# 123-code/Distributed-neural-networks

Hardware: AMD Instinct MI355X
Metric: images/sec CIFAR-10 2-stage (higher is better)
Workload: dtype fp32 (bf16x3 split emulation, ~2^-16 per product); 1 GPU; model=cifar10-convnet (cifar_model_parts.py NeuralNetwork), global_batch=65536, parallelism=pp2-colocated, stages=2, microbatches=1, stage0_spare_cus=0, p2p=none, stage_cut=conv|fc (reference split, 16 KiB/img hop)

## Files before the change

### csrc/bindings.cpp

```cpp
#include <pybind11/pybind11.h>
#include <pybind11/stl.h>
#include <hip/hip_runtime.h>
#include <cstdint>

#include "kernels/api.h"
#include "comm/p2p.h"

#include <string>
#include <vector>

namespace py = pybind11;
#define P(x) reinterpret_cast<void*>(static_cast<uintptr_t>(x))
#define CP(x) reinterpret_cast<const void*>(static_cast<uintptr_t>(x))
#define FP(x) reinterpret_cast<float*>(static_cast<uintptr_t>(x))
#define CFP(x) reinterpret_cast<const float*>(static_cast<uintptr_t>(x))
#define IP(x) reinterpret_cast<int*>(static_cast<uintptr_t>(x))
#define CIP(x) reinterpret_cast<const int*>(static_cast<uintptr_t>(x))
#define ST(x) reinterpret_cast<hipStream_t>(static_cast<uintptr_t>(x))
typedef uint64_t u64;

PYBIND11_MODULE(_dnn_hip, m) {
  m.doc() = "distributed_neural_networks_amd HIP/CDNA4 kernels (gfx950)";
  m.attr("arch") = "gfx950";

// ... 43 lines not shown
                         P(part), part_cap, ST(st));
  });
  m.def("gemm_rowstats", [](u64 out, int out_ld, u64 in, int in_ld) {
    return dnn_gemm_rowstats(reinterpret_cast<void*>(static_cast<uintptr_t>(out)), out_ld, CP(in), in_ld);
  });
  m.def("gemm_rowstats_written", []() { return dnn_gemm_rowstats_written(); });
  m.def("gemm_set_epi_prefetch", [](int on) { return dnn_gemm_set_epi_prefetch(on); });
  m.def("gemm_oneshot_ablate", [](u64 A, int lda, u64 Wsh, u64 sw, u64 C, int ldc, int M, int N, int K, int cfg,
                                  int abl, u64 st) {
    return dnn_gemm_oneshot_ablate(CP(A), lda, CP(Wsh), CFP(sw), P(C), ldc, M, N, K, cfg, abl, ST(st));
  });
  m.def("quant_fp8_mx", [](u64 x, int ldx, u64 q, int ldq, u64 sx, int M, int K, int kpad, u64 st) {
    return dnn_quant_fp8_mx(CP(x), ldx, P(q), ldq, P(sx), M, K, kpad, ST(st));
  });
  m.def("layernorm_q8_mx", [](u64 x, int ldx, u64 w, u64 b, u64 q, int ldq, u64 sx, int M, int N, int kpad, float eps,
                              int rms, u64 st) {
    return dnn_layernorm_q8_mx(CP(x), ldx, CFP(w), CFP(b), P(q), ldq, P(sx), M, N, kpad, eps, rms, ST(st));
  });
  m.def("gemm_fp8_mx", [](u64 a, u64 sx, u64 w, u64 sw, u64 c, int ldc, u64 bias, u64 r, int ldr, int M, int N, int Kb,
                          int act, u64 qo, int ldq, u64 sxo, int kpo, u64 st) {
    return dnn_gemm_fp8_mx(CP(a), CP(sx), CP(w), CFP(sw), P(c), ldc, CFP(bias), CP(r), ldr, M, N, Kb, act, P(qo), ldq,
                           P(sxo), kpo, ST(st));
  });
  m.def("gemm_fp8_qkv_scatter_mx", [](u64 a, u64 sx, u64 w, u64 sw, u64 bias, u64 q, u64 kc, u64 vc, u64 pos, int B,
                                      int T, int H, int Hkv, int hd, int S, int Kb, u64 st) {
    return dnn_gemm_fp8_qkv_scatter_mx(CP(a), CP(sx), CP(w), CFP(sw), CFP(bias), P(q), P(kc), P(vc),
                                       reinterpret_cast<const int*>(static_cast<uintptr_t>(pos)), B, T, H, Hkv, hd, S,
                                       Kb, ST(st));
  });
  m.def("argmax_final", [](u64 part, int S, int M, u64 out, u64 out2, u64 pos_inc, u64 st, u64 hist, int hist_ld) {
    return dnn_argmax_final(CP(part), S, M, IP(out), IP(out2), IP(pos_inc), ST(st), IP(hist), hist_ld);
  });
  m.def("gemm_oneshot_sweep", [](u64 A, int lda, u64 Wsh, u64 sw, u64 C, int ldc, int M, int N, int K, int mt, int ntw,
                                 int steps, int splitk, int w8, u64 ws, long long ws_bytes, u64 st) {
    return dnn_gemm_oneshot_sweep(CP(A), lda, CP(Wsh), CFP(sw), P(C), ldc, M, N, K, mt, ntw, steps, splitk, w8, P(ws),
                                  ws_bytes, ST(st));
  });
  m.def("gemm_skinny_sweep", [](u64 A, int lda, u64 W, int ldw, u64 sw, u64 C, int ldc, int M, int N, int K, int nt,
                                int u, int ks, int pipe, int w8, u64 st) {
    return dnn_gemm_skinny_sweep(CP(A), lda, CP(W), ldw, CFP(sw), P(C), ldc, M, N, K, nt, u, ks, pipe, w8, ST(st));
  });
  m.def("gemm_set_tile", [](int tile) { return dnn_gemm_set_tile(tile); });
  m.def("gemm_set_anatomy", [](int bits) { return dnn_gemm_set_anatomy(bits); });
  m.def("gemm_set_skinny_pin", [](int id, int ks, int n, int k) { return dnn_gemm_set_skinny_pin(id, ks, n, k); });
  m.def("gemm_set_half_cost", [](float c) { return dnn_gemm_set_half_cost(c); });
  m.def("gemm_bf16_qkv_scatter", [](u64 A, int lda, u64 W, int ldw, u64 bias, u64 rowstat, u64 colsum, u64 q, u64 kc,
                                    u64 vc, u64 pos, int B, int T, int H, int Hkv, int hd, int S, int K, u64 st) {
    return dnn_gemm_bf16_qkv_scatter(CP(A), lda, CP(W), ldw, CFP(bias), CFP(rowstat), CFP(colsum), P(q), P(kc), P(vc),
                                     CIP(pos), B, T, H, Hkv, hd, S, K, ST(st));
  });
  m.def("gemm_fp8_qkv_scatter", [](u64 A8, u64 sa, u64 W8, u64 sw, u64 bias, u64 q, u64 kc, u64 vc, u64 pos, int B,
                                   int T, int H, int Hkv, int hd, int S, int Kb, u64 st) {
    return dnn_gemm_fp8_qkv_scatter(CP(A8), CFP(sa), CP(W8), CFP(sw), CFP(bias), P(q), P(kc), P(vc), CIP(pos), B, T, H,
                                    Hkv, hd, S, Kb, ST(st));
  });
  m.def("gemm_set_res_prefetch", [](int on) { return dnn_gemm_set_res_prefetch(on); });
  m.def("gemm_set_skinny_max_m", [](int m) { return dnn_gemm_set_skinny_max_m(m); });
  m.def("gemm_fp8_set_tile", [](int tile) { return dnn_gemm_fp8_set_tile(tile); });
  m.def("silu_mul_packed", [](u64 gu, int ld_in, u64 out, int ld_out, int M, int F, u64 st) {
    return dnn_silu_mul_packed(CP(gu), ld_in, P(out), ld_out, M, F, ST(st));
  });
  m.def("cifar_stage0_v4", [](u64 x, u64 out, u64 w1p, u64 b1, u64 w2p, u64 b2, int B, int grid, u64 st) {
    return dnn_cifar_stage0_v4(CFP(x), P(out), CP(w1p), CFP(b1), CP(w2p), CFP(b2), B, grid, ST(st));
  });
  m.def("cifar_set_v4_pt", [](int pt) { return dnn_cifar_set_v4_pt(pt); });
  m.def("cifar_stage0_x3", [](u64 x, u64 out, u64 w1h, u64 w1l, u64 b1, u64 w2h, u64 w2l, u64 b2, int B, int grid,
                              u64 st, int split_out) {
    return dnn_cifar_stage0_x3(CFP(x), FP(out), CP(w1h), CP(w1l), CFP(b1), CP(w2h), CP(w2l), CFP(b2), B, grid,
                               ST(st), split_out);
  }, py::arg("x"), py::arg("out"), py::arg("w1h"), py::arg("w1l"), py::arg("b1"), py::arg("w2h"), py::arg("w2l"),
        py::arg("b2"), py::arg("B"), py::arg("grid"), py::arg("st"), py::arg("split_out") = 0);
  m.def("cifar_s0_set_wide_store", [](int on) { return dnn_cifar_s0_set_wide_store(on); });
  m.def("cifar_s0_set_mfma", [](int v) { return dnn_cifar_s0_set_mfma(v); });
  m.def("cifar_s0_get_mfma", []() { return dnn_cifar_s0_get_mfma(); });
  m.def("cifar_split3", [](u64 a, int lda, u64 o, int ldo, int M, int K, u64 st, int blocked) {
    return dnn_cifar_split3(CFP(a), lda, P(o), ldo, M, K, ST(st), blocked);
  }, py::arg("a"), py::arg("lda"), py::arg("o"), py::arg("ldo"), py::arg("M"), py::arg("K"), py::arg("st"),
        py::arg("blocked") = 0);
  m.def("cifar_fc1_x3", [](u64 a, int lda, u64 wh, u64 wl, int ldw, u64 bias, u64 c, int ldc, int M, int N, int K,
                           u64 st, int a_split) {
    return dnn_cifar_fc1_x3(CFP(a), lda, CP(wh), CP(wl), ldw, CFP(bias), FP(c), ldc, M, N, K, ST(st), a_split);
  }, py::arg("a"), py::arg("lda"), py::arg("wh"), py::arg("wl"), py::arg("ldw"), py::arg("bias"), py::arg("c"),
        py::arg("ldc"), py::arg("M"), py::arg("N"), py::arg("K"), py::arg("st"), py::arg("a_split") = 0);
  m.def("cifar_split_blocked", [](u64 a, u64 o, int M, int K, int dir, u64 st) {
    return dnn_cifar_split_blocked(CFP(a), FP(o), M, K, dir, ST(st));
  });
  m.def("cifar_head_tail_x3", [](u64 hid, u64 w2h, u64 w2l, u64 b2, u64 probs, u64 pred, int B, u64 st) {
    return dnn_cifar_head_tail_x3(CFP(hid), CP(w2h), CP(w2l), CFP(b2), FP(probs), IP(pred), B, ST(st));
  });
  m.def("cifar_head_tail", [](u64 hid, u64 w2p, u64 b2, u64 probs, u64 pred, int B, u64 st) {
    return dnn_cifar_head_tail(CP(hid), CP(w2p), CFP(b2), FP(probs), IP(pred), B, ST(st));
  });
#ifdef DNN_HAVE_TRANSFORMER
  m.def("row_stats", [](u64 x, int ldx, u64 stats, int M, int N, float eps, int rms, u64 st) {
    return dnn_row_stats(CP(x), ldx, FP(stats), M, N, eps, rms, ST(st));
  });
  m.def("layernorm", [](u64 x, int ldx, u64 w, u64 b, u64 y, int ldy, int M, int N, float eps, int rms, u64 st) {
    return dnn_layernorm(CP(x), ldx, CFP(w), CFP(b), P(y), ldy, M, N, eps, rms, ST(st));
  });
  m.def("layernorm_q8", [](u64 x, int ldx, u64 w, u64 b, u64 q, int ldq, u64 sq, int M, int N, int kpad, float eps,
                           int rms, u64 st, int split) {
    return dnn_layernorm_q8(CP(x), ldx, CFP(w), CFP(b), P(q), ldq, FP(sq), M, N, kpad, eps, rms, ST(st), split);
  }, py::arg("x"), py::arg("ldx"), py::arg("w"), py::arg("b"), py::arg("q"), py::arg("ldq"), py::arg("sq"), py::arg("M"),
     py::arg("N"), py::arg("kpad"), py::arg("eps"), py::arg("rms"), py::arg("st"), py::arg("split") = 0);
  m.def("embed_gpt2", [](u64 idx, u64 wte, u64 wpe, u64 out, int B, int T, int d, u64 pos, int V, int Pn, u64 st) {
    return dnn_embed_gpt2(CIP(idx), CP(wte), CP(wpe), P(out), B, T, d, CIP(pos), V, Pn, ST(st));
  });
  m.def("qkv_split", [](u64 qkv, u64 q, u64 kc, u64 vc, int B, int T, int H, int Hkv, int hd, int S, u64 pos,
                        u64 cos, u64 sin, int rope, u64 st, int kv8) {
    return dnn_qkv_split(CP(qkv), P(q), P(kc), P(vc), B, T, H, Hkv, hd, S, CIP(pos), CFP(cos), CFP(sin), rope,
                         ST(st), kv8);
  }, py::arg("qkv"), py::arg("q"), py::arg("kc"), py::arg("vc"), py::arg("B"), py::arg("T"), py::arg("H"),
     py::arg("Hkv"), py::arg("hd"), py::arg("S"), py::arg("pos"), py::arg("cos"), py::arg("sin"), py::arg("rope"),
     py::arg("st"), py::arg("kv8") = 0);
  m.def("flash_attn_qkv", [](u64 qkv, int ldqkv, u64 kc, u64 vc, u64 o, int B, int T, int H, int Hkv, int hd, int S,
                             u64 pos, float scale, u64 st, int kv8) {
    return dnn_flash_attn_qkv(CP(qkv), ldqkv, P(kc), P(vc), P(o), B, T, H, Hkv, hd, S, CIP(pos), scale, ST(st), kv8);
  }, py::arg("qkv"), py::arg("ldqkv"), py::arg("kc"), py::arg("vc"), py::arg("o"), py::arg("B"), py::arg("T"),
     py::arg("H"), py::arg("Hkv"), py::arg("hd"), py::arg("S"), py::arg("pos"), py::arg("scale"), py::arg("st"),
     py::arg("kv8") = 0);
  m.def("flash_attn", [](u64 q, u64 kc, u64 vc, u64 o, int B, int T, int H, int Hkv, int hd, int S, u64 pos,
                         float scale, u64 st, int kv8) {
    return dnn_flash_attn(CP(q), CP(kc), CP(vc), P(o), B, T, H, Hkv, hd, S, CIP(pos), scale, ST(st), kv8);
  }, py::arg("q"), py::arg("kc"), py::arg("vc"), py::arg("o"), py::arg("B"), py::arg("T"), py::arg("H"),
     py::arg("Hkv"), py::arg("hd"), py::arg("S"), py::arg("pos"), py::arg("scale"), py::arg("st"), py::arg("kv8") = 0);
  m.def("attn_decode", [](u64 q, u64 kc, u64 vc, u64 o, int B, int H, int Hkv, int hd, int S, u64 lens,
                          float scale, int splits, u64 ws, u64 st, int kv8) {
    return dnn_attn_decode(CP(q), CP(kc), CP(vc), P(o), B, H, Hkv, hd, S, CIP(lens), scale, splits, FP(ws), ST(st),
                           kv8);
  }, py::arg("q"), py::arg("kc"), py::arg("vc"), py::arg("o"), py::arg("B"), py::arg("H"), py::arg("Hkv"),
     py::arg("hd"), py::arg("S"), py::arg("lens"), py::arg("scale"), py::arg("splits"), py::arg("ws"), py::arg("st"),
     py::arg("kv8") = 0);
  m.def("attn_decode_qkv", [](u64 qkv, int ldqkv, u64 kc, u64 vc, u64 o, int B, int H, int Hkv, int hd, int S,
                              u64 pos, u64 cos, u64 sin, float scale, int splits, u64 ws, u64 st, int kv8) {
    return dnn_attn_decode_qkv(CP(qkv), ldqkv, P(kc), P(vc), P(o), B, H, Hkv, hd, S, CIP(pos), CFP(cos), CFP(sin),
                               scale, splits, FP(ws), ST(st), kv8);
  }, py::arg("qkv"), py::arg("ldqkv"), py::arg("kc"), py::arg("vc"), py::arg("o"), py::arg("B"), py::arg("H"),
     py::arg("Hkv"), py::arg("hd"), py::arg("S"), py::arg("pos"), py::arg("cos"), py::arg("sin"), py::arg("scale"),
     py::arg("splits"), py::arg("ws"), py::arg("st"), py::arg("kv8") = 0);
  m.def("sample_topk", [](u64 x, int ld, int M, int N, u64 out, float temperature, int topk, unsigned seed, u64 step,
                          u64 st) {
    return dnn_sample_topk(CP(x), ld, M, N, reinterpret_cast<int*>(out), temperature, topk, seed,
                           reinterpret_cast<const int*>(step), ST(st));
  });
  m.def("sample_rows", [](u64 x, int ld, int M, int N, u64 out, float temperature, int topk, float top_p, float min_p,
                          unsigned seed, u64 step, u64 st, u64 out2, u64 pos_inc, u64 hist, int hist_ld, u64 thr_out) {
    return dnn_sample_rows(CP(x), ld, M, N, IP(out), temperature, topk, top_p, min_p, seed,
                           reinterpret_cast<const int*>(step), ST(st), IP(out2), IP(pos_inc), IP(hist), hist_ld,
                           IP(thr_out));
  }, py::arg("x"), py::arg("ld"), py::arg("M"), py::arg("N"), py::arg("out"), py::arg("temperature"), py::arg("topk"),
     py::arg("top_p"), py::arg("min_p"), py::arg("seed"), py::arg("step"), py::arg("st"), py::arg("out2") = 0,
     py::arg("pos_inc") = 0, py::arg("hist") = 0, py::arg("hist_ld") = 0, py::arg("thr_out") = 0);
  m.def("argmax_rows", [](u64 x, int ld, int M, int N, u64 out, int f32in, u64 st, u64 out2, u64 pos_inc, u64 part,
                          u64 hist, int hist_ld) {
    return dnn_argmax_rows(CP(x), ld, M, N, IP(out), f32in, ST(st), IP(out2), IP(pos_inc),
                           reinterpret_cast<void*>(static_cast<uintptr_t>(part)), IP(hist), hist_ld);
  }, py::arg("x"), py::arg("ld"), py::arg("M"), py::arg("N"), py::arg("out"), py::arg("f32in"), py::arg("st"),
     py::arg("out2") = 0, py::arg("pos_inc") = 0, py::arg("part") = 0, py::arg("hist") = 0, py::arg("hist_ld") = 0);
  m.def("quant_fp8_rows", [](u64 x, int ldx, u64 q, u64 scale, int M, int K, int kpad, u64 st, int split) {
    return dnn_quant_fp8_rows(CP(x), ldx, P(q), FP(scale), M, K, kpad, ST(st), split);
  }, py::arg("x"), py::arg("ldx"), py::arg("q"), py::arg("scale"), py::arg("M"), py::arg("K"), py::arg("kpad"),
     py::arg("st"), py::arg("split") = 0);
  m.def("gemm_fp8", [](u64 A, u64 sa, u64 W, u64 sw, u64 C, int ldc, u64 bias, u64 R, int ldr, int M, int N, int K,
                       int act, u64 st) {
    return dnn_gemm_fp8(CP(A), CFP(sa), CP(W), CFP(sw), P(C), ldc, CFP(bias), CP(R), ldr, M, N, K, act, ST(st));
  });
// ... 48 lines not shown
```

### csrc/kernels/api.h

```cpp
#pragma once
#include <hip/hip_runtime.h>

extern "C" {
int dnn_gemm_bf16(const void* A, int lda, const void* W, int ldw, void* C, int ldc, const float* bias, const void* R,
                  int ldr, int M, int N, int K, int act, int out_f32, hipStream_t st, const void* Wsh = nullptr,
                  const float* rowstat = nullptr, const float* colsum = nullptr, void* ws = nullptr,
                  long long ws_bytes = 0);
int dnn_row_stats(const void* x, int ldx, float* stats, int M, int N, float eps, int rms, hipStream_t st);
int dnn_gemm_set_tile(int tile);
int dnn_gemm_set_anatomy(int bits);
int dnn_gemm_set_skinny_pin(int id, int ks, int n, int k);
int dnn_gemm_bf16_qkv_scatter(const void* A, int lda, const void* W, int ldw, const float* bias, const float* rowstat,
                              const float* colsum, void* q, void* kc, void* vc, const int* pos, int B, int T, int H,
                              int Hkv, int hd, int S, int K, hipStream_t st);
int dnn_gemm_fp8_qkv_scatter(const void* A8, const float* sa, const void* W8, const float* sw, const float* bias,
                             void* q, void* kc, void* vc, const int* pos, int B, int T, int H, int Hkv, int hd, int S,
                             int Kb, hipStream_t st);
int dnn_gemm_set_res_prefetch(int on);
int dnn_gemm_set_half_cost(float c);
int dnn_gemm_set_skinny_max_m(int m);
int dnn_gemm_fp8_set_tile(int tile);
int dnn_gemm_fp8_256(const void* A, const float* sa, const void* W, const float* sw, void* C, int ldc, const float* bias,
                     const void* R, int ldr, int M, int N, int Kb, int act, hipStream_t st);
int dnn_gemm_skinny_sweep(const void* A, int lda, const void* W, int ldw, const float* sw, void* C, int ldc, int M,
                          int N, int K, int nt, int u, int ks, int pipe, int w8, hipStream_t st);
int dnn_gemm_skinny_norm(const void* A, int lda, const void* W, int ldw, void* C, int ldc, const float* bias,
                         const void* R, int ldr, int M, int N, int K, int act, int norm, const float* colsum, float eps,
                         hipStream_t st, const void* Wsh = nullptr, void* ws = nullptr, long long ws_bytes = 0);
int dnn_gemm_skinny_w8(const void* A, int lda, const void* W, int ldw, const float* sw, void* C, int ldc,
                       const float* bias, const void* R, int ldr, int M, int N, int K, int act, int norm,
                       const float* colsum, float eps, hipStream_t st, const void* Wsh = nullptr, void* ws = nullptr,
                       long long ws_bytes = 0);
int dnn_gemm_skinny(const void* A, int lda, const float* sa, const void* W, int ldw, const float* sw, void* C, int ldc,
                    const float* bias, const void* R, int ldr, int M, int N, int K, int act, int out_f32, int fp8,
                    hipStream_t st, const void* Wsh = nullptr, void* ws = nullptr, long long ws_bytes = 0);
int dnn_gemm_set_stream(int on, long long min_bytes, int fold = -1);
int dnn_gemm_set_oneshot(int on, int mt, int ntw, int steps, int splitk);
int dnn_gemm_set_oneshot_lds_floor(int bytes);
int dnn_gemm_set_oneshot_probe(void* rec, int abl);
int dnn_gemm_oneshot_sweep(const void* A, int lda, const void* Wsh, const float* sw, void* C, int ldc, int M, int N,
                           int K, int mt, int ntw, int steps, int splitk, int w8, void* ws, long long ws_bytes,
                           hipStream_t st);
int dnn_gemm_set_head(int on);
int dnn_gemm_head(const void* A, int lda, const void* Wsh, const float* sw, const float* colsum, const float* bias,
                  float eps, int norm, void* C, int ldc, int M, int N, int K, int w8, void* part, int part_cap,
                  hipStream_t st);
int dnn_argmax_final(const void* part, int S, int M, int* out, int* out2, int* pos_inc, hipStream_t st,
                     int* hist = nullptr, int hist_ld = 0);
int dnn_gemm_set_split_tail(int on);
int dnn_quant_fp8_mx(const void* x, int ldx, void* q, int ldq, void* sx, int M, int K, int kpad, hipStream_t st);
int dnn_layernorm_q8_mx(const void* x, int ldx, const float* w, const float* b, void* q, int ldq, void* sx, int M,
                        int N, int kpad, float eps, int rms, hipStream_t st);
int dnn_gemm_fp8_mx(const void* A8, const void* sx, const void* W8, const float* sw, void* C, int ldc,
                    const float* bias, const void* R, int ldr, int M, int N, int Kb, int act, void* qo, int ldq,
                    void* sxo, int kpo, hipStream_t st);
int dnn_gemm_fp8_qkv_scatter_mx(const void* A8, const void* sx, const void* W8, const float* sw, const float* bias,
                                void* q, void* kc, void* vc, const int* pos, int B, int T, int H, int Hkv, int hd,
                                int S, int Kb, hipStream_t st);
int dnn_gemm_rowstats(void* out, int out_ld, const void* in, int in_ld);
int dnn_gemm_rowstats_written();
int dnn_gemm_set_epi_prefetch(int on);
int dnn_gemm_oneshot_ablate(const void* A, int lda, const void* Wsh, const float* sw, void* C, int ldc, int M, int N,
                            int K, int cfg, int abl, hipStream_t st);
int dnn_silu_mul_packed(const void* gu, int ld_in, void* out, int ld_out, int M, int F, hipStream_t st);
int dnn_cifar_stage0_v4(const float* x, void* out, const void* w1p, const float* b1, const void* w2p, const float* b2,
                        int B, int grid, hipStream_t st);
int dnn_cifar_set_v4_pt(int pt);
int dnn_cifar_stage0_x3(const float* x, float* out, const void* w1h, const void* w1l, const float* b1, const void* w2h,
                        const void* w2l, const float* b2, int B, int grid, hipStream_t st, int split_out = 0);
int dnn_cifar_s0_set_wide_store(int on);
int dnn_cifar_s0_set_mfma(int v);
int dnn_cifar_s0_get_mfma();
int dnn_cifar_split3(const float* a, int lda, void* o, int ldo, int M, int K, hipStream_t st, int blocked = 0);
int dnn_cifar_fc1_x3(const float* A, int lda, const void* Wh, const void* Wl, int ldw, const float* bias, float* C,
                     int ldc, int M, int N, int K, hipStream_t st, int a_split = 0);
int dnn_cifar_split_blocked(const float* a, float* o, int M, int K, int dir, hipStream_t st);
int dnn_cifar_head_tail_x3(const float* hid, const void* w2h, const void* w2l, const float* b2, float* probs, int* pred,
                           int B, hipStream_t st);
int dnn_cifar_head_tail(const void* hid, const void* w2p, const float* b2, float* probs, int* pred, int B,
                        hipStream_t st);
int dnn_layernorm_q8(const void* x, int ldx, const float* w, const float* b, void* q, int ldq, float* sq, int M, int N,
                     int kpad, float eps, int rms, hipStream_t st, int split = 0);
int dnn_layernorm(const void* x, int ldx, const float* w, const float* b, void* y, int ldy, int M, int N, float eps,
                  int rms, hipStream_t st);
int dnn_embed_gpt2(const int* idx, const void* wte, const void* wpe, void* out, int B, int T, int d, const int* pos,
                   int V, int P, hipStream_t st);
int dnn_qkv_split(const void* qkv, void* q, void* kc, void* vc, int B, int T, int H, int Hkv, int hd, int S,
                  const int* pos, const float* cos, const float* sin, int rope, hipStream_t st, int kv8 = 0);
int dnn_flash_attn_qkv(const void* qkv, int ldqkv, void* kc, void* vc, void* o, int B, int T, int H, int Hkv,
                       int hd, int S, const int* pos, float scale, hipStream_t st, int kv8 = 0);
int dnn_flash_attn(const void* q, const void* kc, const void* vc, void* o, int B, int T, int H, int Hkv, int hd, int S,
                   const int* pos, float scale, hipStream_t st, int kv8 = 0);
int dnn_attn_decode_qkv(const void* qkv, int ldqkv, void* kc, void* vc, void* o, int B, int H, int Hkv, int hd, int S,
                        const int* pos, const float* cosT, const float* sinT, float scale, int splits, float* ws,
                        hipStream_t st, int kv8 = 0);
int dnn_attn_decode(const void* q, const void* kc, const void* vc, void* o, int B, int H, int Hkv, int hd, int S,
                    const int* lens, float scale, int splits, float* ws, hipStream_t st, int kv8 = 0);
int dnn_sample_topk(const void* x, int ld, int M, int N, int* out, float temperature, int topk, unsigned seed,
                    const int* step, hipStream_t st);
int dnn_sample_rows(const void* x, int ld, int M, int N, int* out, float temperature, int topk, float top_p,
                    float min_p, unsigned seed, const int* step, hipStream_t st, int* out2 = nullptr,
                    int* pos_inc = nullptr, int* hist = nullptr, int hist_ld = 0, int* thr_out = nullptr);
int dnn_argmax_rows(const void* x, int ld, int M, int N, int* out, int f32in, hipStream_t st, int* out2 = nullptr,
                    int* pos_inc = nullptr, void* part = nullptr, int* hist = nullptr, int hist_ld = 0);
int dnn_quant_fp8_rows(const void* x, int ldx, void* q, float* scale, int M, int K, int kpad, hipStream_t st,
                       int split = 0);
int dnn_gemm_fp8(const void* A, const float* sa, const void* W, const float* sw, void* C, int ldc, const float* bias,
                 const void* R, int ldr, int M, int N, int K, int act, hipStream_t st);
}
```

### csrc/kernels/cifar_x3.hip

```cpp
#include <type_traits>

#include "gemm_epilogue.h"

namespace dnn {
namespace x3 {

__device__ __forceinline__ void split2(float a, float b, uint32_t& hi, uint32_t& lo) {
  hi = pack2bf(a, b);
  const float ah = __uint_as_float(hi << 16), bh = __uint_as_float(hi & 0xffff0000u);
  lo = pack2bf(a - ah, b - bh);
}

__device__ __forceinline__ int dpp_xor1(int v) { return __builtin_amdgcn_mov_dpp(v, 0xB1, 0xF, 0xF, false); }
__device__ __forceinline__ int dpp_xor2(int v) { return __builtin_amdgcn_mov_dpp(v, 0x4E, 0xF, 0xF, false); }

constexpr int XW = 40;
constexpr int XPL = 34 * XW * 8;
constexpr int A1PL = 18 * 18 * 64;
constexpr int A1_OFF = 4 * XPL;
constexpr int LDS_BYTES = A1_OFF + 4 * A1PL;

__device__ __forceinline__ int xin_off(int k, int lo) { return ((k & 1) * 2 + lo) * XPL; }
__device__ __forceinline__ int a1_off(int k, int lo) { return A1_OFF + ((k & 1) * 2 + lo) * A1PL; }

// ... 324 lines not shown
#pragma unroll
          for (int par = 0; par < 2; ++par) b[ky][par] = rb + lb[ky][par];
        f32x16 acc[2] = {f32x16{}, f32x16{}};
        bf16x8 a0[4], a1[4];
        c2_issue<0>(b, a0);
        c2_step<0>(b, w2hf, w2lf, acc, a0, a1);
        if constexpr (WIDE) {
#pragma unroll
          for (int qy = 0; qy < 2; ++qy) {
            const int g0 = (2 * qy) * 4;
            float v[2][2];
#pragma unroll
            for (int i = 0; i < 2; ++i) {
              v[i][0] = fmaxf(fmax_nan(fmax_nan(acc[i][g0], acc[i][g0 + 1]), fmax_nan(acc[i][g0 + 4], acc[i][g0 + 5])) + bias, 0.f);
              v[i][1] = fmaxf(fmax_nan(fmax_nan(acc[i][g0 + 2], acc[i][g0 + 3]), fmax_nan(acc[i][g0 + 6], acc[i][g0 + 7])) + bias,
                              0.f);
            }
            const auto sx = __builtin_amdgcn_permlane32_swap(__float_as_uint(v[0][0]), __float_as_uint(v[1][0]), false,
                                                             false);
            const auto sy = __builtin_amdgcn_permlane32_swap(__float_as_uint(v[0][1]), __float_as_uint(v[1][1]), false,
                                                             false);
            const int PY = 2 * ty2 + qy;
            if constexpr (SPLIT_OUT) {
              uint2 hi, lo;
              split2(__uint_as_float(sx[0]), __uint_as_float(sy[0]), hi.x, lo.x);
              split2(__uint_as_float(sx[1]), __uint_as_float(sy[1]), hi.y, lo.y);
              char* bp = reinterpret_cast<char*>(ob - oc2 * 64) + (oc2 * 2 + (PY >> 2)) * 128 + ((PY & 3) * 8 + 4 * h) * 2;
              *reinterpret_cast<uint2*>(bp) = hi;
              *reinterpret_cast<uint2*>(bp + 64) = lo;
            } else {
              *reinterpret_cast<uint4*>(ob + PY * 8 + 4 * h) = make_uint4(sx[0], sy[0], sx[1], sy[1]);
            }
          }
        } else {
#pragma unroll
        for (int i = 0; i < 2; ++i) {
#pragma unroll
          for (int qy = 0; qy < 2; ++qy) {
            float2 pv;
            const int g0 = (2 * qy) * 4;
            pv.x = fmaxf(fmax_nan(fmax_nan(acc[i][g0], acc[i][g0 + 1]), fmax_nan(acc[i][g0 + 4], acc[i][g0 + 5])) + bias, 0.f);
            pv.y = fmaxf(fmax_nan(fmax_nan(acc[i][g0 + 2], acc[i][g0 + 3]), fmax_nan(acc[i][g0 + 6], acc[i][g0 + 7])) + bias,
                         0.f);
            const int PY = 2 * ty2 + qy, PX = 4 * i + 2 * h;
            if constexpr (SPLIT_OUT) {
              uint32_t hi, lo;
              split2(pv.x, pv.y, hi, lo);
              char* bp = reinterpret_cast<char*>(ob - oc2 * 64) + (oc2 * 2 + (PY >> 2)) * 128 + ((PY & 3) * 8 + PX) * 2;
              *reinterpret_cast<uint32_t*>(bp) = hi;
              *reinterpret_cast<uint32_t*>(bp + 64) = lo;
            } else {
              *reinterpret_cast<float2*>(ob + PY * 8 + PX) = pv;
            }
          }
        }
        }
      }
    };

    __syncthreads();
    for (int it = 0; it <= n; ++it) {
      if (it >= 1) conv2_img(it - 1);
      __syncthreads();
    }
  }
}

constexpr int F1_T = 256, F1_K = 32, F1_PLANE = 256 * 64;

__device__ __forceinline__ int f1_swz(int r) { return (r >> 2) & 2; }

__device__ __forceinline__ bf16x8 f1_frag(const char* plane, int row, int chunk) {
  return *reinterpret_cast<const bf16x8*>(plane + row * 64 + ((chunk ^ f1_swz(row)) << 4));
}

__device__ __forceinline__ void f1_tile_coords(int logical, int ntm, int ntn, int& tm, int& tn) {
  constexpr int G = 8;
  const int per = G * ntn, grp = logical / per, first = grp * G;
  const int gm = min(ntm - first, G), r = logical - grp * per;
  tm = first + r % gm;
  tn = r / gm;
}

template <bool SPLIT_IN>
__global__ __launch_bounds__(512, 1) void cifar_fc1_x3_kernel(const float* __restrict__ A, int lda,
                                                              const bf16_t* __restrict__ Wh,
                                                              const bf16_t* __restrict__ Wl, int ldw,
                                                              const float* __restrict__ bias, float* __restrict__ C,
                                                              int ldc, int M, int N, int K) {
  __shared__ __attribute__((aligned(1024))) char smem[2 * 4 * F1_PLANE];
  const int tid = threadIdx.x, lane = tid & 63, wave = tid >> 6;
  const int ntn = N / F1_T, ntm = (M + F1_T - 1) / F1_T;
  int tm, tn;
  f1_tile_coords(xcd_remap(blockIdx.x, ntm * ntn), ntm, ntn, tm, tn);
  const int m0 = tm * F1_T, n0 = tn * F1_T;
  const int wr = wave >> 2, wc = wave & 3;
  const int nk = K / F1_K;
  auto plane = [&](int u, int p) { return smem + (u * 4 + p) * F1_PLANE; };

  float4 ar[4];
  auto load_a = [&](int t, auto) {
#pragma unroll
    for (int k = 0; k < 4; ++k) {
      const int row = min(m0 + (tid >> 3) + 64 * k, M - 1);
      ar[k] = *reinterpret_cast<const float4*>(A + (size_t)row * lda + t * F1_K + (tid & 7) * 4);
    }
  };
  auto store_a = [&](int u, auto) {
#pragma unroll
    for (int k = 0; k < 4; ++k) {
      const int r = (tid >> 3) + 64 * k, c = (tid & 7) >> 1, half = tid & 1;
      uint2 hi, lo;
      split2(ar[k].x, ar[k].y, hi.x, lo.x);
      split2(ar[k].z, ar[k].w, hi.y, lo.y);
      const int o = r * 64 + ((c ^ f1_swz(r)) << 4) + half * 8;
      *reinterpret_cast<uint2*>(plane(u, 0) + o) = hi;
      *reinterpret_cast<uint2*>(plane(u, 1) + o) = lo;
    }
  };
  auto stage_a = [&](int u, int t) {
    const char* Ab = reinterpret_cast<const char*>(A);
#pragma unroll
    for (int p = 0; p < 2; ++p) {
#pragma unroll
      for (int j = 0; j < 2; ++j) {
        const int piece = wave * 2 + j, rl = piece * 16 + (lane >> 2);
        const int c = (lane & 3) ^ f1_swz(rl);
        const int row = min(m0 + rl, M - 1);
        glds16(Ab + (size_t)row * lda * 4 + t * 128 + p * 64 + c * 16, plane(u, p) + piece * 1024);
      }
    }
  };
  auto stage_w = [&](int u, int t) {
#pragma unroll
    for (int p = 0; p < 2; ++p) {
      const bf16_t* W = p ? Wl : Wh;
#pragma unroll
      for (int j = 0; j < 2; ++j) {
        const int piece = wave * 2 + j, rl = piece * 16 + (lane >> 2);
        const int c = (lane & 3) ^ f1_swz(rl);
        glds16(W + (size_t)(n0 + rl) * ldw + t * F1_K + c * 8, plane(u, 2 + p) + piece * 1024);
      }
    }
  };

  f32x4 acc[8][4];
#pragma unroll
  for (int i = 0; i < 8; ++i)
#pragma unroll
    for (int j = 0; j < 4; ++j) acc[i][j] = f32x4{0.f, 0.f, 0.f, 0.f};

  using I0 = std::integral_constant<int, 0>;
  if constexpr (SPLIT_IN) {
    stage_a(0, 0);
    stage_w(0, 0);
    asm volatile("s_waitcnt vmcnt(0)" ::: "memory");
  } else {
    load_a(0, I0{});
    stage_w(0, 0);
    asm volatile("s_waitcnt vmcnt(0)" ::: "memory");
    store_a(0, I0{});
  }
  __syncthreads();

  const int fr = lane & 15, fc = lane >> 4;
  auto compute = [&](int u) {
    const char* ah_p = plane(u, 0);
    const char* al_p = plane(u, 1);
    const char* bh_p = plane(u, 2);
    const char* bl_p = plane(u, 3);
    bf16x8 bh[4], bl[4];
#pragma unroll
    for (int j = 0; j < 4; ++j) {
      bh[j] = f1_frag(bh_p, wc * 64 + j * 16 + fr, fc);
      bl[j] = f1_frag(bl_p, wc * 64 + j * 16 + fr, fc);
    }
#pragma unroll
    for (int h = 0; h < 2; ++h) {
      bf16x8 ah[4], al[4];
#pragma unroll
      for (int i = 0; i < 4; ++i) {
        ah[i] = f1_frag(ah_p, wr * 128 + (h * 4 + i) * 16 + fr, fc);
        al[i] = f1_frag(al_p, wr * 128 + (h * 4 + i) * 16 + fr, fc);
      }
#pragma unroll
      for (int i = 0; i < 4; ++i)
#pragma unroll
        for (int j = 0; j < 4; ++j) {
          f32x4& a = acc[h * 4 + i][j];
          a = __builtin_amdgcn_mfma_f32_16x16x32_bf16(bh[j], ah[i], a, 0, 0, 0);
          a = __builtin_amdgcn_mfma_f32_16x16x32_bf16(bl[j], ah[i], a, 0, 0, 0);
          a = __builtin_amdgcn_mfma_f32_16x16x32_bf16(bh[j], al[i], a, 0, 0, 0);
        }
    }
  };
  auto barrier = [&]() {
    asm volatile("s_waitcnt lgkmcnt(0)" ::: "memory");
    __builtin_amdgcn_sched_barrier(0);
    __builtin_amdgcn_s_barrier();
    __builtin_amdgcn_sched_barrier(0);
  };
  for (int t = 0; t < nk; ++t) {
    const int u = t & 1;
    if (t + 1 < nk) {
      if constexpr (SPLIT_IN)
        stage_a(u ^ 1, t + 1);
      else
        load_a(t + 1, I0{});
      stage_w(u ^ 1, t + 1);
    }
    compute(u);
    if (t + 1 < nk) {
      asm volatile("s_waitcnt vmcnt(0)" ::: "memory");
      if constexpr (!SPLIT_IN) store_a(u ^ 1, I0{});
    }
    barrier();
  }

  const bool vec = epi_vec_ok(C, ldc, bias, nullptr, 0);
#pragma unroll
  for (int i = 0; i < 8; ++i) {
    const int m = m0 + wr * 128 + i * 16 + fr;
#pragma unroll
    for (int j = 0; j < 4; ++j)
      epi_t4<ACT_RELU, true>(acc[i][j], m, n0 + wc * 64 + j * 16 + fc * 4, M, N, C, ldc, bias, nullptr, 0, vec);
  }
}

__global__ __launch_bounds__(256) void cifar_split_blocked_kernel(const float* __restrict__ a, float* __restrict__ o,
                                                                  int M, int K, int dir) {
  const int per_row = K / 8;
  const long total = (long)M * per_row;
  for (long e = blockIdx.x * 256L + threadIdx.x; e < total; e += (long)gridDim.x * 256) {
    const int m = (int)(e / per_row), k = (int)(e % per_row) * 8;
    char* rowp = reinterpret_cast<char*>(o + (size_t)m * K);
    const char* rowa = reinterpret_cast<const char*>(a + (size_t)m * K);
    const int hoff = (k >> 5) * 128 + (k & 31) * 2;
    if (dir == 0) {
      const float4 u = *reinterpret_cast<const float4*>(rowa + k * 4);
      const float4 v = *reinterpret_cast<const float4*>(rowa + k * 4 + 16);
      uint4 hi, lo;
      split2(u.x, u.y, hi.x, lo.x);
      split2(u.z, u.w, hi.y, lo.y);
      split2(v.x, v.y, hi.z, lo.z);
      split2(v.z, v.w, hi.w, lo.w);
      *reinterpret_cast<uint4*>(rowp + hoff) = hi;
      *reinterpret_cast<uint4*>(rowp + hoff + 64) = lo;
    } else {
      const uint4 hi = *reinterpret_cast<const uint4*>(rowa + hoff);
      const uint4 lo = *reinterpret_cast<const uint4*>(rowa + hoff + 64);
      const uint32_t h[4] = {hi.x, hi.y, hi.z, hi.w}, l[4] = {lo.x, lo.y, lo.z, lo.w};
      float r[8];
#pragma unroll
      for (int i = 0; i < 4; ++i) {
        r[2 * i] = __uint_as_float(h[i] << 16) + __uint_as_float(l[i] << 16);
        r[2 * i + 1] = __uint_as_float(h[i] & 0xffff0000u) + __uint_as_float(l[i] & 0xffff0000u);
      }
      *reinterpret_cast<float4*>(rowp + k * 4) = float4{r[0], r[1], r[2], r[3]};
      *reinterpret_cast<float4*>(rowp + k * 4 + 16) = float4{r[4], r[5], r[6], r[7]};
    }
  }
}

__global__ __launch_bounds__(256) void cifar_split3_kernel(const float* __restrict__ a, int lda,
                                                           bf16_t* __restrict__ o, int ldo, int M, int K,
                                                           int blocked) {
  const int per_row = K / 8;
  const long total = (long)M * per_row;
  for (long e = blockIdx.x * 256L + threadIdx.x; e < total; e += (long)gridDim.x * 256) {
    const int m = (int)(e / per_row), c = (int)(e % per_row) * 8;
    uint4 hi, lo;
    if (blocked) {
      const char* rowa = reinterpret_cast<const char*>(a + (size_t)m * lda) + (c >> 5) * 128 + (c & 31) * 2;
      hi = *reinterpret_cast<const uint4*>(rowa);
      lo = *reinterpret_cast<const uint4*>(rowa + 64);
    } else {
      const float4 u = *reinterpret_cast<const float4*>(a + (size_t)m * lda + c);
      const float4 v = *reinterpret_cast<const float4*>(a + (size_t)m * lda + c + 4);
      split2(u.x, u.y, hi.x, lo.x);
      split2(u.z, u.w, hi.y, lo.y);
      split2(v.x, v.y, hi.z, lo.z);
      split2(v.z, v.w, hi.w, lo.w);
    }
    bf16_t* r = o + (size_t)m * ldo + c;
    *reinterpret_cast<uint4*>(r) = hi;
    *reinterpret_cast<uint4*>(r + K) = hi;
    *reinterpret_cast<uint4*>(r + 2 * K) = lo;
  }
}

__global__ __launch_bounds__(256) void cifar_head_tail_x3_kernel(const float* __restrict__ hid,
                                                                 const bf16_t* __restrict__ w2h,
                                                                 const bf16_t* __restrict__ w2l,
                                                                 const float* __restrict__ b2,
                                                                 float* __restrict__ probs, int* __restrict__ pred,
                                                                 int B) {
  const int lane = threadIdx.x & 63;
  const int gw = (blockIdx.x * blockDim.x + threadIdx.x) >> 6;
  const int nw = (gridDim.x * blockDim.x) >> 6;
// ... 11 lines not shown
    const float* ap = hid + (size_t)rc * 512 + kq;
    f32x4 acc = {0.f, 0.f, 0.f, 0.f};
#pragma unroll
    for (int s = 0; s < 16; ++s) {
      const float4 u = *reinterpret_cast<const float4*>(ap + s * 32);
      const float4 v = *reinterpret_cast<const float4*>(ap + s * 32 + 4);
      uint4 hi, lo;
      split2(u.x, u.y, hi.x, lo.x);
      split2(u.z, u.w, hi.y, lo.y);
      split2(v.x, v.y, hi.z, lo.z);
      split2(v.z, v.w, hi.w, lo.w);
      const bf16x8 ah = __builtin_bit_cast(bf16x8, hi), al = __builtin_bit_cast(bf16x8, lo);
      acc = __builtin_amdgcn_mfma_f32_16x16x32_bf16(ah, wfh[s], acc, 0, 0, 0);
      acc = __builtin_amdgcn_mfma_f32_16x16x32_bf16(ah, wfl[s], acc, 0, 0, 0);
      acc = __builtin_amdgcn_mfma_f32_16x16x32_bf16(al, wfh[s], acc, 0, 0, 0);
    }
#pragma unroll
    for (int r = 0; r < 4; ++r) {
      const float z = col < 10 ? acc[r] + bias : -INFINITY;
      float mx = z;
#pragma unroll
      for (int o = 1; o < 16; o <<= 1) mx = fmaxf(mx, __shfl_xor(mx, o, 64));
      const float e = col < 10 ? expf(z - mx) : 0.f;
      float sum = e;
#pragma unroll
      for (int o = 1; o < 16; o <<= 1) sum += __shfl_xor(sum, o, 64);
      int cand = (z == mx) ? col : 16;
#pragma unroll
      for (int o = 1; o < 16; o <<= 1) cand = min(cand, __shfl_xor(cand, o, 64));
      const int m = r0 + (lane >> 4) * 4 + r;
      if (m < B) {
        if (col < 10) probs[(size_t)m * 10 + col] = e / sum;
        if (col == 0) pred[m] = cand;
      }
    }
  }
}

}

using namespace dnn;

static int g_s0_wide_store = 1;
static int g_s0_mfma = 1;

extern "C" int dnn_cifar_s0_set_mfma(int v) {
  if (v < 0 || v > 1) return 1;
  g_s0_mfma = v;
  return 0;
}

extern "C" int dnn_cifar_s0_get_mfma() { return g_s0_mfma; }

extern "C" int dnn_cifar_s0_set_wide_store(int on) {
  g_s0_wide_store = on ? 1 : 0;
  return 0;
}

template <bool SPLIT_OUT>
static int launch_stage0_x3(const float* x, float* out, const void* w1h, const void* w1l, const float* b1,
                            const void* w2h, const void* w2l, const float* b2, int B, int grid, hipStream_t st) {
  if (g_s0_mfma == 1)
    hipLaunchKernelGGL((cifar_stage0_x3_kernel<true, SPLIT_OUT, 1>), dim3(grid), dim3(512), 0, st, x, out,
                       (const bf16_t*)w1h, (const bf16_t*)w1l, b1, (const bf16_t*)w2h, (const bf16_t*)w2l, b2, B);
  else if (g_s0_wide_store)
    hipLaunchKernelGGL((cifar_stage0_x3_kernel<true, SPLIT_OUT>), dim3(grid), dim3(512), 0, st, x, out,
                       (const bf16_t*)w1h, (const bf16_t*)w1l, b1, (const bf16_t*)w2h, (const bf16_t*)w2l, b2, B);
  else
    hipLaunchKernelGGL((cifar_stage0_x3_kernel<false, SPLIT_OUT>), dim3(grid), dim3(512), 0, st, x, out,
                       (const bf16_t*)w1h, (const bf16_t*)w1l, b1, (const bf16_t*)w2h, (const bf16_t*)w2l, b2, B);
  return (int)hipGetLastError();
}

extern "C" int dnn_cifar_stage0_x3(const float* x, float* out, const void* w1h, const void* w1l, const float* b1,
                                   const void* w2h, const void* w2l, const float* b2, int B, int grid,
                                   hipStream_t st, int split_out) {
  if (B <= 0) return 0;
  if (grid <= 0) grid = 256;
  if (grid > B) grid = B;
  return split_out ? launch_stage0_x3<true>(x, out, w1h, w1l, b1, w2h, w2l, b2, B, grid, st)
                   : launch_stage0_x3<false>(x, out, w1h, w1l, b1, w2h, w2l, b2, B, grid, st);
}

extern "C" int dnn_cifar_fc1_x3(const float* A, int lda, const void* Wh, const void* Wl, int ldw, const float* bias,
                                float* C, int ldc, int M, int N, int K, hipStream_t st, int a_split) {
  if (M <= 0) return 0;
  if (N % F1_T != 0 || K % F1_K != 0 || lda % 4 != 0 || ldw % 8 != 0 || ldc % 4 != 0) return -1;
  const int blocks = ((M + F1_T - 1) / F1_T) * (N / F1_T);
  if (a_split)
    hipLaunchKernelGGL(cifar_fc1_x3_kernel<true>, dim3(blocks), dim3(512), 0, st, A, lda, (const bf16_t*)Wh,
                       (const bf16_t*)Wl, ldw, bias, C, ldc, M, N, K);
  else
    hipLaunchKernelGGL(cifar_fc1_x3_kernel<false>, dim3(blocks), dim3(512), 0, st, A, lda, (const bf16_t*)Wh,
                       (const bf16_t*)Wl, ldw, bias, C, ldc, M, N, K);
  return (int)hipGetLastError();
}

extern "C" int dnn_cifar_split_blocked(const float* a, float* o, int M, int K, int dir, hipStream_t st) {
  if (M <= 0) return 0;
  if (K % 32 != 0 || a == o) return -1;
  const long total = (long)M * (K / 8);
  long blocks = (total + 255) / 256;
  if (blocks > 8192) blocks = 8192;
  hipLaunchKernelGGL(cifar_split_blocked_kernel, dim3((int)blocks), dim3(256), 0, st, a, o, M, K, dir);
  return (int)hipGetLastError();
}

extern "C" int dnn_cifar_split3(const float* a, int lda, void* o, int ldo, int M, int K, hipStream_t st, int blocked) {
  if (M <= 0) return 0;
  if (K % 8 != 0 || lda % 4 != 0 || ldo % 8 != 0 || ldo < 3 * K || (blocked && K % 32 != 0)) return -1;
  const long total = (long)M * (K / 8);
  long blocks = (total + 255) / 256;
  if (blocks > 8192) blocks = 8192;
  hipLaunchKernelGGL(cifar_split3_kernel, dim3((int)blocks), dim3(256), 0, st, a, lda, (bf16_t*)o, ldo, M, K, blocked);
  return (int)hipGetLastError();
}

extern "C" int dnn_cifar_head_tail_x3(const float* hid, const void* w2h, const void* w2l, const float* b2,
                                      float* probs, int* pred, int B, hipStream_t st) {
  if (B <= 0) return 0;
  int waves = (B + 15) / 16;
  int blocks = (waves + 3) / 4;
  if (blocks > 1024) blocks = 1024;
  hipLaunchKernelGGL(cifar_head_tail_x3_kernel, dim3(blocks), dim3(256), 0, st, hid, (const bf16_t*)w2h,
                     (const bf16_t*)w2l, b2, probs, pred, B);
  return (int)hipGetLastError();
}
```

### distributed_neural_networks_amd/ops/cifar.py

```python
from __future__ import annotations

from dataclasses import dataclass
from typing import Dict, Optional, Tuple

import torch

from ._lib import check, lib, ptr, stream_ptr
from .gemm import ACT_RELU, linear

PRECISIONS = ("fp32", "bf16")


def split_bf16(w: torch.Tensor) -> Tuple[torch.Tensor, torch.Tensor]:
    w = w.float()
    hi = w.to(torch.bfloat16)
    lo = (w - hi.float()).to(torch.bfloat16)
    return hi, lo


def _conv1_k48(sd) -> torch.Tensor:
    w = torch.zeros(32, 3, 4, 4)
    w[:, :, :3, :3] = sd["conv1.weight"].float().permute(0, 2, 3, 1)
    return w.reshape(32, 48)

# ... 21 lines not shown
    w2l: torch.Tensor = None


@dataclass
class CifarHeadWeights:
    precision: str
    w_fc1: torch.Tensor = None
    w_fc1h: torch.Tensor = None
    w_fc1l: torch.Tensor = None
    b_fc1: torch.Tensor = None
    w_fc2: torch.Tensor = None
    w_fc2h: torch.Tensor = None
    w_fc2l: torch.Tensor = None
    b_fc2: torch.Tensor = None


def _check_precision(p: str) -> str:
    if p not in PRECISIONS:
        raise ValueError(f"CIFAR precision must be one of {PRECISIONS}, got {p!r}")
    return p


def pack_stage0(sd: Dict[str, torch.Tensor], device, precision: str = "fp32") -> CifarStage0Weights:
    _check_precision(precision)
    b1 = sd["conv1.bias"].float().to(device).contiguous()
    b2 = sd["conv2.bias"].float().to(device).contiguous()
    w1, w2 = _conv1_k48(sd), _conv2_k288(sd)
    if precision == "bf16":
        return CifarStage0Weights("bf16", b1, b2,
                                  w1=w1.to(device=device, dtype=torch.bfloat16).contiguous(),
                                  w2=w2.to(device=device, dtype=torch.bfloat16).contiguous())
    (w1h, w1l), (w2h, w2l) = split_bf16(w1), split_bf16(w2)
    dv = lambda t: t.to(device).contiguous()
    return CifarStage0Weights("fp32", b1, b2, w1h=dv(w1h), w1l=dv(w1l), w2h=dv(w2h), w2l=dv(w2l))


def pack_head(sd: Dict[str, torch.Tensor], device, fc1: bool = True, fc2: bool = True,
              precision: str = "fp32") -> CifarHeadWeights:
    _check_precision(precision)
    w = CifarHeadWeights(precision)
    if fc1:
        f = sd["fc1.weight"].float()
        if precision == "bf16":
            w.w_fc1 = f.to(device=device, dtype=torch.bfloat16).contiguous()
        else:
            hi, lo = split_bf16(f)
            w.w_fc1 = torch.cat([hi, lo, hi], dim=1).to(device).contiguous()
            w.w_fc1h, w.w_fc1l = hi.to(device).contiguous(), lo.to(device).contiguous()
        w.b_fc1 = sd["fc1.bias"].float().to(device).contiguous()
    if fc2:
        f2 = _fc2_pad(sd)
        if precision == "bf16":
            w.w_fc2 = f2.to(device=device, dtype=torch.bfloat16).contiguous()
        else:
            hi, lo = split_bf16(f2)
            w.w_fc2h, w.w_fc2l = hi.to(device).contiguous(), lo.to(device).contiguous()
        w.b_fc2 = sd["fc2.bias"].float().to(device).contiguous()
    return w


def act_dtype(precision: str) -> torch.dtype:
    return torch.float32 if _check_precision(precision) == "fp32" else torch.bfloat16


STAGE0_GRID = 0
FC1_X3_MIN_ROWS = 16384


def set_stage0_grid(grid: int = 0) -> None:
    global STAGE0_GRID
    STAGE0_GRID = int(grid)


STAGE0_MFMA = {"32x32x16": 0, "16x16x32": 1}


def set_stage0_mfma(shape) -> int:
    v = STAGE0_MFMA[shape] if isinstance(shape, str) else int(shape)
    prev = lib().cifar_s0_get_mfma()
    check(lib().cifar_s0_set_mfma(v), "cifar_s0_set_mfma")
    return prev


def _check_act(t: torch.Tensor, shape, dtype, what: str) -> None:
    if t.dtype != dtype or tuple(t.shape[1:]) != tuple(shape) or not t.is_contiguous():
        raise ValueError(f"{what}: expected contiguous {dtype} (B,{','.join(map(str, shape))}), "
                         f"got {t.dtype} {tuple(t.shape)}")


BOUNDARIES = ("fp32", "split")


def _split_boundary(boundary: str, precision: str) -> int:
    if boundary not in BOUNDARIES:
        raise ValueError(f"boundary must be one of {BOUNDARIES}, got {boundary!r}")
    if boundary == "split" and precision != "fp32":
        raise ValueError("the split boundary encoding exists for the fp32 precision only")
    return int(boundary == "split")


def encode_boundary(h: torch.Tensor, out: Optional[torch.Tensor] = None) -> torch.Tensor:
    out = torch.empty_like(h) if out is None else out
    check(lib().cifar_split_blocked(ptr(h), ptr(out), h.shape[0], h.shape[1], 0, stream_ptr()), "encode_boundary")
    return out


def decode_boundary(h: torch.Tensor, out: Optional[torch.Tensor] = None) -> torch.Tensor:
    out = torch.empty_like(h) if out is None else out
    check(lib().cifar_split_blocked(ptr(h), ptr(out), h.shape[0], h.shape[1], 1, stream_ptr()), "decode_boundary")
    return out


def stage0_forward(x: torch.Tensor, w: CifarStage0Weights, out: Optional[torch.Tensor] = None,
                   grid: int = 0, boundary: str = "fp32") -> torch.Tensor:
    split = _split_boundary(boundary, w.precision)
    grid = grid or STAGE0_GRID
    _check_act(x, (3, 32, 32), torch.float32, "stage0 input")
    B = x.shape[0]
    dt = act_dtype(w.precision)
    if out is None:
        out = torch.empty((B, 4096), dtype=dt, device=x.device)
    if tuple(out.shape) != (B, 4096) or out.dtype != dt or not out.is_contiguous():
        raise ValueError("stage0: bad output buffer")
    if w.precision == "fp32":
        check(lib().cifar_stage0_x3(ptr(x), ptr(out), ptr(w.w1h), ptr(w.w1l), ptr(w.b1), ptr(w.w2h), ptr(w.w2l),
                                    ptr(w.b2), B, grid, stream_ptr(), split), "cifar_stage0_x3")
    else:
        check(lib().cifar_stage0_v4(ptr(x), ptr(out), ptr(w.w1), ptr(w.b1), ptr(w.w2), ptr(w.b2), B, grid,
                                    stream_ptr()), "cifar_stage0_v4")
    return out


def fc1_forward(h: torch.Tensor, w: CifarHeadWeights, out: Optional[torch.Tensor] = None,
                scratch: Optional[torch.Tensor] = None, boundary: str = "fp32") -> torch.Tensor:
    split = _split_boundary(boundary, w.precision)
    dt = act_dtype(w.precision)
    _check_act(h, (4096,), dt, "fc1 input")
    B = h.shape[0]
    if w.precision == "bf16":
        return linear(h, w.w_fc1, w.b_fc1, act=ACT_RELU, out=out)
    if B >= FC1_X3_MIN_ROWS:
        if out is None:
            out = torch.empty((B, 512), dtype=torch.float32, device=h.device)
        check(lib().cifar_fc1_x3(ptr(h), 4096, ptr(w.w_fc1h), ptr(w.w_fc1l), 4096, ptr(w.b_fc1), ptr(out), 512,
                                 B, 512, 4096, stream_ptr(), split), "cifar_fc1_x3")
        return out
    if scratch is None or scratch.shape[0] < B or tuple(scratch.shape[1:]) != (3 * 4096,):
        scratch = torch.empty((B, 3 * 4096), dtype=torch.bfloat16, device=h.device)
    a3 = scratch[:B]
    check(lib().cifar_split3(ptr(h), 4096, ptr(a3), 3 * 4096, B, 4096, stream_ptr(), split), "cifar_split3")
    if out is None:
        out = torch.empty((B, 512), dtype=torch.float32, device=h.device)
    return linear(a3, w.w_fc1, w.b_fc1, act=ACT_RELU, out=out)


def head_tail(hid: torch.Tensor, w: CifarHeadWeights, probs: Optional[torch.Tensor] = None,
              pred: Optional[torch.Tensor] = None) -> Tuple[torch.Tensor, torch.Tensor]:
    _check_act(hid, (512,), act_dtype(w.precision), "head_tail input")
    B = hid.shape[0]
    probs = probs if probs is not None else torch.empty((B, 10), dtype=torch.float32, device=hid.device)
    pred = pred if pred is not None else torch.empty((B,), dtype=torch.int32, device=hid.device)
    if w.precision == "fp32":
        check(lib().cifar_head_tail_x3(ptr(hid), ptr(w.w_fc2h), ptr(w.w_fc2l), ptr(w.b_fc2), ptr(probs), ptr(pred),
                                       B, stream_ptr()), "cifar_head_tail_x3")
    else:
        check(lib().cifar_head_tail(ptr(hid), ptr(w.w_fc2), ptr(w.b_fc2), ptr(probs), ptr(pred), B, stream_ptr()),
# ... 10 lines not shown
```

Before: 28.37 million images/s.

## Stagger fc1 x3 kernel wave groups so DMA staging overlaps MFMA compute

Adds a staggered schedule for the fc1 bf16x3 GEMM kernel. The two wave-row groups are offset by one phase: one group issues the next tile's global loads while the other runs its MFMA segment. Fragments are read into registers before the barrier, and the A tile is prefetched two steps ahead. The aim is to hide global-load and LDS latency behind matrix-core work, at the cost of more registers and tricky barrier and waitcnt ordering. The new schedule is on by default and can be switched back at runtime.

New measurement: 28.87 million images/s (median of 6 runs). +1.8%, better.

```diff
diff --git a/csrc/bindings.cpp b/csrc/bindings.cpp
--- a/csrc/bindings.cpp
+++ b/csrc/bindings.cpp
@@ -149,6 +149,8 @@
     return dnn_cifar_fc1_x3(CFP(a), lda, CP(wh), CP(wl), ldw, CFP(bias), FP(c), ldc, M, N, K, ST(st), a_split);
   }, py::arg("a"), py::arg("lda"), py::arg("wh"), py::arg("wl"), py::arg("ldw"), py::arg("bias"), py::arg("c"),
         py::arg("ldc"), py::arg("M"), py::arg("N"), py::arg("K"), py::arg("st"), py::arg("a_split") = 0);
+  m.def("cifar_fc1_set_sched", [](int v) { return dnn_cifar_fc1_set_sched(v); });
+  m.def("cifar_fc1_get_sched", []() { return dnn_cifar_fc1_get_sched(); });
   m.def("cifar_split_blocked", [](u64 a, u64 o, int M, int K, int dir, u64 st) {
     return dnn_cifar_split_blocked(CFP(a), FP(o), M, K, dir, ST(st));
   });
diff --git a/csrc/kernels/api.h b/csrc/kernels/api.h
--- a/csrc/kernels/api.h
+++ b/csrc/kernels/api.h
@@ -74,6 +74,8 @@
 int dnn_cifar_split3(const float* a, int lda, void* o, int ldo, int M, int K, hipStream_t st, int blocked = 0);
 int dnn_cifar_fc1_x3(const float* A, int lda, const void* Wh, const void* Wl, int ldw, const float* bias, float* C,
                      int ldc, int M, int N, int K, hipStream_t st, int a_split = 0);
+int dnn_cifar_fc1_set_sched(int v);
+int dnn_cifar_fc1_get_sched();
 int dnn_cifar_split_blocked(const float* a, float* o, int M, int K, int dir, hipStream_t st);
 int dnn_cifar_head_tail_x3(const float* hid, const void* w2h, const void* w2l, const float* b2, float* probs, int* pred,
                            int B, hipStream_t st);
diff --git a/csrc/kernels/cifar_x3.hip b/csrc/kernels/cifar_x3.hip
--- a/csrc/kernels/cifar_x3.hip
+++ b/csrc/kernels/cifar_x3.hip
@@ -430,7 +430,7 @@
   tn = r / gm;
 }
 
-template <bool SPLIT_IN>
+template <bool SPLIT_IN, bool STAG = false>
 __global__ __launch_bounds__(512, 1) void cifar_fc1_x3_kernel(const float* __restrict__ A, int lda,
                                                               const bf16_t* __restrict__ Wh,
                                                               const bf16_t* __restrict__ Wl, int ldw,
@@ -446,18 +446,21 @@
   const int nk = K / F1_K;
   auto plane = [&](int u, int p) { return smem + (u * 4 + p) * F1_PLANE; };
 
+  int ltid = tid;
   float4 ar[4];
   auto load_a = [&](int t, auto) {
+    const int x = ltid;
 #pragma unroll
     for (int k = 0; k < 4; ++k) {
-      const int row = min(m0 + (tid >> 3) + 64 * k, M - 1);
-      ar[k] = *reinterpret_cast<const float4*>(A + (size_t)row * lda + t * F1_K + (tid & 7) * 4);
+      const int row = min(m0 + (x >> 3) + 64 * k, M - 1);
+      ar[k] = *reinterpret_cast<const float4*>(A + (size_t)row * lda + t * F1_K + (x & 7) * 4);
     }
   };
   auto store_a = [&](int u, auto) {
+    const int x = ltid;
 #pragma unroll
     for (int k = 0; k < 4; ++k) {
-      const int r = (tid >> 3) + 64 * k, c = (tid & 7) >> 1, half = tid & 1;
+      const int r = (x >> 3) + 64 * k, c = (x & 7) >> 1, half = x & 1;
       uint2 hi, lo;
       split2(ar[k].x, ar[k].y, hi.x, lo.x);
       split2(ar[k].z, ar[k].w, hi.y, lo.y);
@@ -468,6 +471,7 @@
   };
   auto stage_a = [&](int u, int t) {
     const char* Ab = reinterpret_cast<const char*>(A);
+    const int lane = ltid & 63, wave = ltid >> 6;
 #pragma unroll
     for (int p = 0; p < 2; ++p) {
 #pragma unroll
@@ -480,6 +484,7 @@
     }
   };
   auto stage_w = [&](int u, int t) {
+    const int lane = ltid & 63, wave = ltid >> 6;
 #pragma unroll
     for (int p = 0; p < 2; ++p) {
       const bf16_t* W = p ? Wl : Wh;
@@ -508,8 +513,18 @@
     stage_w(0, 0);
     asm volatile("s_waitcnt vmcnt(0)" ::: "memory");
     store_a(0, I0{});
-  }
-  __syncthreads();
+    if constexpr (STAG) {
+      if (nk > 1) load_a(1, I0{});
+    }
+  }
+  if constexpr (STAG) {
+    asm volatile("s_waitcnt lgkmcnt(0)" ::: "memory");
+    __builtin_amdgcn_sched_barrier(0);
+    __builtin_amdgcn_s_barrier();
+    __builtin_amdgcn_sched_barrier(0);
+  } else {
+    __syncthreads();
+  }
 
   const int fr = lane & 15, fc = lane >> 4;
   auto compute = [&](int u) {
@@ -548,21 +563,90 @@
     __builtin_amdgcn_s_barrier();
     __builtin_amdgcn_sched_barrier(0);
   };
-  for (int t = 0; t < nk; ++t) {
-    const int u = t & 1;
-    if (t + 1 < nk) {
-      if constexpr (SPLIT_IN)
-        stage_a(u ^ 1, t + 1);
+  if constexpr (!STAG) {
+    for (int t = 0; t < nk; ++t) {
+      const int u = t & 1;
+      if (t + 1 < nk) {
+        if constexpr (SPLIT_IN)
+          stage_a(u ^ 1, t + 1);
+        else
+          load_a(t + 1, I0{});
+        stage_w(u ^ 1, t + 1);
+      }
+      compute(u);
+      if (t + 1 < nk) {
+        asm volatile("s_waitcnt vmcnt(0)" ::: "memory");
+        if constexpr (!SPLIT_IN) store_a(u ^ 1, I0{});
+      }
+      barrier();
+    }
+  } else {
+    bf16x8 fbh[4], fbl[4], fah[8], fal[8];
+    auto read_frags = [&](int u) {
+      const int fr = ltid & 15, fc = (ltid >> 4) & 3, wc = (ltid >> 6) & 3, wr = ltid >> 8;
+#pragma unroll
+      for (int j = 0; j < 4; ++j) {
+        fbh[j] = f1_frag(plane(u, 2), wc * 64 + j * 16 + fr, fc);
+        fbl[j] = f1_frag(plane(u, 3), wc * 64 + j * 16 + fr, fc);
+      }
+#pragma unroll
+      for (int i = 0; i < 8; ++i) {
+        fah[i] = f1_frag(plane(u, 0), wr * 128 + i * 16 + fr, fc);
+        fal[i] = f1_frag(plane(u, 1), wr * 128 + i * 16 + fr, fc);
+      }
+    };
+    auto mfma_seg = [&]() {
+      __builtin_amdgcn_sched_barrier(0);
+#pragma unroll
+      for (int i = 0; i < 8; ++i)
+#pragma unroll
+        for (int term = 0; term < 3; ++term)
+#pragma unroll
+          for (int j = 0; j < 4; ++j)
+            acc[i][j] = __builtin_amdgcn_mfma_f32_16x16x32_bf16(term == 1 ? fbl[j] : fbh[j], term == 2 ? fal[i] : fah[i],
+                                                                acc[i][j], 0, 0, 0);
+      __builtin_amdgcn_sched_barrier(0);
+    };
+    auto retire_dma = [&](bool a_in_flight) {
+      if (a_in_flight)
+        asm volatile("s_waitcnt vmcnt(4)" ::: "memory");
       else
-        load_a(t + 1, I0{});
-      stage_w(u ^ 1, t + 1);
-    }
-    compute(u);
-    if (t + 1 < nk) {
-      asm volatile("s_waitcnt vmcnt(0)" ::: "memory");
-      if constexpr (!SPLIT_IN) store_a(u ^ 1, I0{});
-    }
-    barrier();
+        asm volatile("s_waitcnt vmcnt(0)" ::: "memory");
+    };
+    auto stage_next = [&](int u, int t) {
+      if constexpr (SPLIT_IN) stage_a(u, t);
+      stage_w(u, t);
+    };
+    const bool g1 = __builtin_amdgcn_readfirstlane(wr) != 0;
+    auto fresh_tid = [&]() {
+      ltid = tid;
+      asm volatile("" : "+v"(ltid));
+    };
+    if (g1) {
+      if (nk > 1) stage_next(1, 1);
+      barrier();
+    }
+    for (int t = 0; t < nk; ++t) {
+      const int u = t & 1;
+      fresh_tid();
+      read_frags(u);
+      if (t + 1 < nk) {
+        if constexpr (!SPLIT_IN) store_a(u ^ 1, I0{});
+        if (!g1) stage_next(u ^ 1, t + 1);
+        if constexpr (!SPLIT_IN) {
+          if (t + 2 < nk) load_a(t + 2, I0{});
+        }
+        if (g1) retire_dma(!SPLIT_IN && t + 2 < nk);
+      }
+      barrier();
+      if (g1 && t + 2 < nk) {
+        fresh_tid();
+        stage_next(u, t + 2);
+      }
+      mfma_seg();
+      if (!g1 && t + 1 < nk) retire_dma(!SPLIT_IN && t + 2 < nk);
+      if (!g1 || t + 1 < nk) barrier();
+    }
   }
 
   const bool vec = epi_vec_ok(C, ldc, bias, nullptr, 0);
@@ -740,18 +824,35 @@
                    : launch_stage0_x3<false>(x, out, w1h, w1l, b1, w2h, w2l, b2, B, grid, st);
 }
 
+static int g_fc1_sched = 1;
+
+extern "C" int dnn_cifar_fc1_set_sched(int v) {
+  if (v < 0 || v > 1) return 1;
+  g_fc1_sched = v;
+  return 0;
+}
+
+extern "C" int dnn_cifar_fc1_get_sched() { return g_fc1_sched; }
+
+template <bool SPLIT_IN>
+static int launch_fc1_x3(const float* A, int lda, const void* Wh, const void* Wl, int ldw, const float* bias, float* C,
+                         int ldc, int M, int N, int K, int blocks, hipStream_t st) {
+  if (g_fc1_sched == 1)
+    hipLaunchKernelGGL((cifar_fc1_x3_kernel<SPLIT_IN, true>), dim3(blocks), dim3(512), 0, st, A, lda,
+                       (const bf16_t*)Wh, (const bf16_t*)Wl, ldw, bias, C, ldc, M, N, K);
+  else
+    hipLaunchKernelGGL((cifar_fc1_x3_kernel<SPLIT_IN, false>), dim3(blocks), dim3(512), 0, st, A, lda,
+                       (const bf16_t*)Wh, (const bf16_t*)Wl, ldw, bias, C, ldc, M, N, K);
+  return (int)hipGetLastError();
+}
+
 extern "C" int dnn_cifar_fc1_x3(const float* A, int lda, const void* Wh, const void* Wl, int ldw, const float* bias,
                                 float* C, int ldc, int M, int N, int K, hipStream_t st, int a_split) {
   if (M <= 0) return 0;
-  if (N % F1_T != 0 || K % F1_K != 0 || lda % 4 != 0 || ldw % 8 != 0 || ldc % 4 != 0) return -1;
+  if (N % F1_T != 0 || K < F1_K || K % F1_K != 0 || lda % 4 != 0 || ldw % 8 != 0 || ldc % 4 != 0) return -1;
   const int blocks = ((M + F1_T - 1) / F1_T) * (N / F1_T);
-  if (a_split)
-    hipLaunchKernelGGL(cifar_fc1_x3_kernel<true>, dim3(blocks), dim3(512), 0, st, A, lda, (const bf16_t*)Wh,
-                       (const bf16_t*)Wl, ldw, bias, C, ldc, M, N, K);
-  else
-    hipLaunchKernelGGL(cifar_fc1_x3_kernel<false>, dim3(blocks), dim3(512), 0, st, A, lda, (const bf16_t*)Wh,
-                       (const bf16_t*)Wl, ldw, bias, C, ldc, M, N, K);
-  return (int)hipGetLastError();
+  return a_split ? launch_fc1_x3<true>(A, lda, Wh, Wl, ldw, bias, C, ldc, M, N, K, blocks, st)
+                 : launch_fc1_x3<false>(A, lda, Wh, Wl, ldw, bias, C, ldc, M, N, K, blocks, st);
 }
 
 extern "C" int dnn_cifar_split_blocked(const float* a, float* o, int M, int K, int dir, hipStream_t st) {
diff --git a/distributed_neural_networks_amd/ops/cifar.py b/distributed_neural_networks_amd/ops/cifar.py
--- a/distributed_neural_networks_amd/ops/cifar.py
+++ b/distributed_neural_networks_amd/ops/cifar.py
@@ -127,6 +127,16 @@
     return prev
 
 
+FC1_SCHED = {"lockstep": 0, "staggered": 1}
+
+
+def set_fc1_sched(sched) -> int:
+    v = FC1_SCHED[sched] if isinstance(sched, str) else int(sched)
+    prev = lib().cifar_fc1_get_sched()
+    check(lib().cifar_fc1_set_sched(v), "cifar_fc1_set_sched")
+    return prev
+
+
 def _check_act(t: torch.Tensor, shape, dtype, what: str) -> None:
     if t.dtype != dtype or tuple(t.shape[1:]) != tuple(shape) or not t.is_contiguous():
         raise ValueError(f"{what}: expected contiguous {dtype} (B,{','.join(map(str, shape))}), "
```
